# DiltheyLab/HLA-LA

Hardware: AMD Instinct MI355X
Metric: paired reads/sec aligned to PRG graph (higher is better)
Workload: dtype int32

## Files before the change

hla-la_amd/csrc/batch.h:

```cpp
#pragma once
#include "device_common.h"

namespace hlala {

template <template <class> class Ptr> struct DevBatchT {
    int n_pairs, n_reads, n_chains, stride;
    int from_seeds;
    int unpaired;
    Ptr<const int> read_off;
    Ptr<const uint8_t> read_bases;
    Ptr<const uint8_t> read_quals;
    Ptr<const int> chain_off;
    Ptr<const int> read_primary;
    Ptr<const int> chain_read;
    Ptr<const int> chain_contig;
    Ptr<const int> chain_pos;
    Ptr<const int> chain_offset;
    Ptr<const int> chain_as;
    Ptr<const uint8_t> chain_reverse;
    Ptr<const int> cigar_off;
    Ptr<const u32> cigar;
    Ptr<int> seed_status;
    Ptr<int> seed_ncols;
    Ptr<int> seed_begin;
// ... 40 lines not shown
    Ptr<int> order_hist;
    int order_shift, order_nb;
    int long_chunk_nodes, long_max_segs;
    int order_cost;
    Ptr<int> chain_row;
    int n_rows;
    Ptr<int> dp_blk;
    Ptr<int> dp_list;
    int dp_nblk;
    int dp_band;
    int dp_band_risky;
    int dp_jf;
    Ptr<void> dp_items;
    Ptr<int> dbg;
};
typedef DevBatchT<HostP> DevBatch;
typedef DevBatchT<GlobP> DevBatchG;
static_assert(sizeof(DevBatch) == sizeof(DevBatchG), "one layout");
__device__ __forceinline__ const DevBatchG& dev_view(const DevBatch* p) { return *(const DevBatchG*)p; }
enum { DESC_VALUE = 0, DESC_VIEW = 1, DESC_GENERIC = 2 };
template <int FORM, class D> __device__ __forceinline__ decltype(auto) desc_of(const D& byValue, const D* inMemory)
{
    if constexpr (FORM == DESC_VIEW) return dev_view(inMemory);
    else if constexpr (FORM == DESC_GENERIC) return (*inMemory);
    else return (byValue);
}

template <class BT> __device__ __forceinline__ int ordered_chains(const BT& B) { return B.chain_order ? __builtin_amdgcn_readfirstlane(B.order_hist[B.order_nb - 1]) : B.n_chains; }

template <class BT> __device__ __forceinline__ size_t row_base(const BT& B, int c) { return (size_t)(B.chain_row ? B.chain_row[c] : c) * (size_t)B.stride; }

enum { DPL_BAND16 = 0, DPL_BAND32 = 2, DPL_BAND64 = 4, DPL_JF = 6, DPL_GEN = 8, DPL_N = 10 };
__host__ __device__ inline int dpl_of_class(int cls) { return cls == 0 ? DPL_GEN : (cls == 1 ? DPL_JF : (cls == 2 ? DPL_BAND16 : (cls == 3 ? DPL_BAND32 : DPL_BAND64))); }
enum { WC_PAIR_MULTI = 40, WC_BAND_FETCH = 48, WC_FO_COUNT = 54, WC_FO_FETCH = 56, WC_BAND_FAILED = 58, WC_BAND_CALLS = 59, WC_JF_FAILED = 60, WC_BAND_WHY = 62, WC_BAND_TIED = 68,
       WC_N = 88 };
constexpr int BAND_MAXJ16 = 15, BAND_MAXJ32 = 31, BAND_MAXJ64 = 48;

enum {
    CNT_CHAINS_EXT = 0, CNT_DP_CALLS, CNT_DP_ITERS, CNT_DP_CELLS, CNT_SEED_COLS, CNT_OUT_COLS, CNT_EDGES, CNT_ERRORS, CNT_DP_SHARED
};

}
```

hla-la_amd/csrc/hlala_api.hip:

```cpp
#include <cmath>
#include <cstdio>
#include <cstring>
#include <cstdlib>
#include <algorithm>
#include <map>
#include <mutex>
#include <chrono>
#include <thread>
#include <set>
#include <string>
#include <unordered_map>
#include <vector>

#include "../../include/hlala_gpu.h"
#include "batch.h"
#include "flat_graph.hpp"
#include "host_internal.h"

#include "kernel_dp.hip"
#include "kernel_project.hip"
#include "kernel_order.hip"
#include "kernel_pair.hip"
#include "kernel_typer.hip"
#include "kernel_call.hip"
// ... 16 lines not shown

struct hlala_ctx {
    int device = 0;
    hipStream_t stream = nullptr;
    hipStream_t side = nullptr;
    hipStream_t up = nullptr, rs = nullptr, active = nullptr;
    int tail_pool_k = 1; std::vector<hlala_batch*> tail;
    hipEvent_t evSideTail = nullptr; bool sideTailValid = false;
    hlala_params params{};
    FlatGraph F;
    DevGraph G{};
    DevGraph* dG = nullptr;
    DevTables* dT = nullptr;
    double* d_islog = nullptr;
    long long* d_contig_off = nullptr; uint8_t* d_contig_seq = nullptr; int* d_contig_level = nullptr;
    int n_contigs = 0; std::vector<long long> contig_off;
    std::vector<void*> allocs;
    std::unordered_map<void*, size_t> block_bytes;
    std::multimap<size_t, void*> pool;
    size_t pool_bytes = 0;
    size_t pool_cap = (size_t)176 << 30;
    std::mutex pool_mu;
    std::set<struct hlala_batch*> batches;
    int jf_margin = 16;
    int stitch_by_row = 1;
    int stitch_draw = 12;
    bool side_after_pair = false;
    bool rows_all = false;
    bool band_risky = false;
    int band_grid = 0, band_margin = 8;
    char* tiny_slabs = nullptr; size_t tiny_slab_bytes = 0; int tiny_grid = 0; int jf_grid = 0;
    char* ext_slabs = nullptr; size_t ext_slab_bytes = 0; char* wide_slabs = nullptr; char* mid_slabs = nullptr; char* large_slabs = nullptr; size_t large_slab_bytes = 0; char* huge_slabs = nullptr; size_t huge_slab_bytes = 0; int huge_grid = 0; int ext_grid = 0; int wide_grid = 0; int broad_grid = 0; int retry_grid = 0; int stitch_grid = 0; int mid_grid = 0; size_t mid_slab_bytes = 0;
    char* proj_slabs = nullptr; size_t proj_slab_bytes = 0; int proj_grid = 0, pair_grid = 0, pair_lean_grid = 0;
    char* rethread_slabs = nullptr; size_t rethread_slab_bytes = 0; int rethread_grid = 0;
    double* pair_scratch = nullptr;
    char* proj_long_slabs = nullptr; size_t proj_long_slab_bytes = 0;
    void* create_scratch = nullptr; size_t create_scratch_bytes = 0; bool create_scratch_pinned = false;
    int long_chunk_nodes = 1 << 20, long_max_segs = 1 << 20;
    int order_cost = 0;
    int order_shift = 8, order_nb = 0;
    int* dbg_host = nullptr;
    int* d_cov = nullptr; int n_cov = 0; int* d_gene_first = nullptr; int* d_gene_last = nullptr; int n_genes = 0;
    struct KeptReads { uint8_t* store = nullptr; long long* start = nullptr; int* length = nullptr; int n = 0; };
    std::vector<KeptReads> kept;
    std::string err;
};

struct hlala_batch {
    hlala_ctx* ctx = nullptr;
    DevBatch B{};
    DevBatch* dB = nullptr;
    std::vector<void*> allocs;
    int staged = 0;
    bool prepared = false;
    int n_rows_host = 0;
    bool outputs_ready = false;
    bool side_used = false;
    bool side_pending = false;
    bool tail_pooled = false;
    bool side_inflight = false;
    hipEvent_t evDone = nullptr;
    hipEvent_t evMain = nullptr; bool mainValid = false;
    hipEvent_t ev[14]{}; hipEvent_t evC[7][2]{}; hipEvent_t evSide[8]{}; hipEvent_t evJF = nullptr;  hipEvent_t evBand[2]{};  bool band_used = false; bool eventsMade = false;
    uint32_t first_chain = 0;
    float ms[3] = {0, 0, 0};
};

// ... 329 lines not shown

    c->wide_grid = cus * 7;
    c->stitch_grid = cus * 20;
    if(const char* e = getenv("HLALA_STITCH_BY_ROW")) c->stitch_by_row = atoi(e) != 0;
    c->ext_slab_bytes = dp_slab_bytes<DpSmall>() > dp_slab_bytes<DpWide>() ? dp_slab_bytes<DpSmall>() : dp_slab_bytes<DpWide>();
    c->large_slab_bytes = dp_slab_bytes<DpLarge>() > dp_slab_bytes<DpBroad>() ? dp_slab_bytes<DpLarge>() : dp_slab_bytes<DpBroad>();
    c->huge_grid = cus / 4 > 0 ? cus / 4 : 1;
    c->huge_slab_bytes = dp_inmemory_bytes<DpHuge>();
    if((rc = slab_pool(&c->tiny_slabs, c->tiny_slab_bytes * (size_t)(64 / DpTiny::GW) * (size_t)std::max(c->tiny_grid, c->jf_grid), "16-lane DP slabs"))) return fail(rc);
    if((rc = slab_pool(&c->mid_slabs, c->mid_slab_bytes * (size_t)(64 / DpMid::GW) * (size_t)c->mid_grid, "32-lane DP slabs"))) return fail(rc);
    if((rc = slab_pool(&c->ext_slabs, c->ext_slab_bytes * (size_t)c->ext_grid, "64-lane DP slabs"))) return fail(rc);
    if((rc = slab_pool(&c->wide_slabs, c->ext_slab_bytes * (size_t)c->wide_grid, "wide-class DP slabs"))) return fail(rc);
    if((rc = slab_pool(&c->large_slabs, c->large_slab_bytes * (size_t)(c->broad_grid + c->retry_grid), "large-class DP slabs"))) return fail(rc);
    if((rc = slab_pool(&c->huge_slabs, c->huge_slab_bytes * (size_t)c->huge_grid, "in-memory DP class"))) return fail(rc);
    c->proj_grid = cus * (c->params.max_columns <= PROJ_CAP_SHORT ? 12 : 8); c->pair_grid = cus * 16; c->pair_lean_grid = cus * 24;
    { int rcp = dev_alloc(c, c->allocs, (size_t)2 * c->pair_grid * PAIR_COMB, &c->pair_scratch, false); if(rcp) return fail(rcp); }
    if(c->params.max_columns > PROJ_CAP) {
        c->proj_grid = cus * 20;
        c->proj_long_slab_bytes = proj_long_slab_bytes();
        c->stitch_draw = 1;
        if(device_malloc_retry(c->device, nullptr, (void**)&c->proj_long_slabs, c->proj_long_slab_bytes * (size_t)c->proj_grid) != hipSuccess) { c->err = "hipMalloc(long-read projection slabs) failed"; return fail(HLALA_E_DEVICE); }
        c->allocs.push_back(c->proj_long_slabs);
    }
    c->proj_slab_bytes = proj_slab_bytes_host(c->params.max_columns, F.max_nodes_per_level);
    if(device_malloc_retry(c->device, nullptr, (void**)&c->proj_slabs, c->proj_slab_bytes * (size_t)c->proj_grid) != hipSuccess) { c->err = "hipMalloc(projection slabs) failed"; return fail(HLALA_E_DEVICE); }
    c->allocs.push_back(c->proj_slabs);
    if(!c->proj_long_slabs) {
        const char* e = getenv("HLALA_RETHREAD");
        if(!(e && atoi(e) == 0)) {
            size_t ent = (size_t)c->params.max_columns * (size_t)RT_SN; if(ent < 1024) ent = 1024;
            c->rethread_slab_bytes = (ent * sizeof(ChoiceRec) + 255) & ~(size_t)255;
            if(c->rethread_slab_bytes > c->proj_slab_bytes) c->rethread_slab_bytes = c->proj_slab_bytes;
            c->rethread_grid = cus * 24;
            if(device_malloc_retry(c->device, nullptr, (void**)&c->rethread_slabs, c->rethread_slab_bytes * (size_t)c->rethread_grid) != hipSuccess) { c->err = "hipMalloc(re-threading slabs) failed"; return fail(HLALA_E_DEVICE); }
            c->allocs.push_back(c->rethread_slabs);
        }
    }
    { const char* e = getenv("HLALA_LOCALITY");
      if(!(e && atoi(e) == 0)) { int sh = 8; if(e && atoi(e) >= 2 && atoi(e) <= 20) sh = atoi(e); while((F.L >> sh) + 2 > 16384) sh++; c->order_shift = sh; c->order_nb = (F.L >> sh) + 2; } }
    if(const char* e = getenv("HLALA_LONG_CHUNK_NODES")) { const int v = atoi(e); if(v >= 1) c->long_chunk_nodes = v; }
    if(const char* e = getenv("HLALA_LONG_MAXSEGS")) { const int v = atoi(e); if(v >= 0) c->long_max_segs = v; }
    if(c->proj_long_slabs && c->order_nb > 0) { const char* e = getenv("HLALA_LONG_ORDER"); c->order_cost = (e && atoi(e) == 0) ? 0 : 1; }
    if(getenv("HLALA_DEBUG")) { if(hipMalloc((void**)&c->dbg_host, 8192 * sizeof(int)) != hipSuccess) c->dbg_host = nullptr; else { (void)hipMemset(c->dbg_host, 0, 8192 * sizeof(int)); c->allocs.push_back(c->dbg_host); } }
    if(hipEventCreateWithFlags(&c->evSideTail, hipEventDisableTiming) != hipSuccess) { c->err = "hipEventCreate failed"; return fail(HLALA_E_DEVICE); }
    { int prLow = 0, prHigh = 0; (void)hipDeviceGetStreamPriorityRange(&prLow, &prHigh);
      if(hipStreamCreateWithPriority(&c->up, hipStreamNonBlocking, prHigh) != hipSuccess || hipStreamCreateWithPriority(&c->rs, hipStreamNonBlocking, prHigh) != hipSuccess ||
         hipStreamCreateWithPriority(&c->side, hipStreamNonBlocking, prLow) != hipSuccess) { c->err = "hipStreamCreate failed"; return fail(HLALA_E_DEVICE); } }
    if(hipStreamSynchronize(c->active) != hipSuccess) { c->err = "upload failed"; return fail(HLALA_E_DEVICE); }
    { std::lock_guard<std::mutex> g(g_ctx_mu); g_ctxs.push_back(c); }
    *out = c;
    return HLALA_OK;
}

void hlala_destroy(hlala_ctx* c)
{
    if(!c) return;
    DEV_GUARD(c);
    { std::lock_guard<std::mutex> g(g_ctx_mu); g_ctxs.erase(std::remove(g_ctxs.begin(), g_ctxs.end(), c), g_ctxs.end()); }
    if(!c->tail.empty()) (void)flush_tail(c);
    for(hlala_batch* b : c->batches) b->ctx = nullptr;
    for(void* p : c->allocs) if(p) (void)hipFree(p);
    if(c->create_scratch) { if(c->create_scratch_pinned) (void)hipHostFree(c->create_scratch); else free(c->create_scratch); }
    for(hlala_ctx::KeptReads& kr : c->kept) { (void)hipFree(kr.store); (void)hipFree(kr.start); (void)hipFree(kr.length); }
    for(auto& kv : c->pool) (void)hipFree(kv.second);
    if(c->side) { (void)hipStreamSynchronize(c->side); (void)hipStreamDestroy(c->side); }
    if(c->up) { (void)hipStreamSynchronize(c->up); (void)hipStreamDestroy(c->up); }
// ... 322 lines not shown
{
    DEV_GUARD(c);
    if(!c || !b) return HLALA_E_ARG;
    { int rj = join_side(c, b); if(rj) return rj; }
    if(b->B.from_seeds) { c->err = "batch was created from seeds: stage A not available"; return HLALA_E_STATE; }
    { int re = batch_events(c, b); if(re) return re; }
    { int ro = ensure_outputs(c, b); if(ro) return ro; }
    DevBatch& B = b->B;
    HIP_TRY(c, hipMemsetAsync(B.work_counter, 0, WC_N * sizeof(int), c->active));
    HIP_TRY(c, hipMemsetAsync(B.counters, 0, 32 * sizeof(u64), c->active));
    HIP_TRY(c, hipEventRecord(b->ev[0], c->active));
    if(B.n_chains > 0) {
        int threads = 256, blocks = (B.n_reads + threads - 1) / threads;
        if(!b->prepared && B.order_hist) HIP_TRY(c, hipMemsetAsync(B.order_hist, 0, ((size_t)B.order_nb + 1) * sizeof(int), c->active));
        if(!b->prepared) hipLaunchKernelGGL(k_filter_chains, dim3(blocks), dim3(threads), 0, c->active, c->dG, b->dB, c->d_contig_off, c->d_contig_level);
        if(!b->prepared && B.order_hist) {
            hipLaunchKernelGGL(k_order_scan, dim3(1), dim3(ORDER_SCAN_THREADS), 0, c->active, B.order_hist, B.order_nb);
            hipLaunchKernelGGL(k_order_scatter, dim3((B.n_chains + 255) / 256), dim3(256), 0, c->active, b->dB);
            int rco = check_launch(c, "k_order_scatter"); if(rco) return rco;
        }
        int grid = B.n_chains < c->proj_grid ? B.n_chains : c->proj_grid;
        if(c->proj_long_slabs)
            hipLaunchKernelGGL((k_project_chains<ProjLdsLong>), dim3(grid), dim3(64), 0, c->active, c->G, b->B, c->dG, b->dB, c->d_contig_off, c->d_contig_seq, c->d_contig_level,
                               c->proj_slabs, c->proj_slab_bytes, c->proj_long_slabs, c->proj_long_slab_bytes, 0);
        else
            if(c->params.max_columns <= PROJ_CAP_SHORT)
                hipLaunchKernelGGL((k_project_chains<ProjLdsShort>), dim3(grid), dim3(64), 0, c->active, c->G, b->B, c->dG, b->dB, c->d_contig_off, c->d_contig_seq, c->d_contig_level,
                                   c->proj_slabs, c->proj_slab_bytes, (char*)nullptr, (size_t)0, c->rethread_slabs ? 1 : 0);
            else
                hipLaunchKernelGGL((k_project_chains<ProjLds>), dim3(grid), dim3(64), 0, c->active, c->G, b->B, c->dG, b->dB, c->d_contig_off, c->d_contig_seq, c->d_contig_level,
                               c->proj_slabs, c->proj_slab_bytes, (char*)nullptr, (size_t)0, c->rethread_slabs ? 1 : 0);
        int rc = check_launch(c, "k_project_chains"); if(rc) return rc;
        if(c->rethread_slabs) {
            hipLaunchKernelGGL(k_rethread_chains, dim3(c->rethread_grid), dim3(64), 0, c->active, c->dG, b->dB, c->rethread_slabs, c->rethread_slab_bytes);
            rc = check_launch(c, "k_rethread_chains"); if(rc) return rc;
        }
    }
    HIP_TRY(c, hipEventRecord(b->ev[1], c->active));
    b->staged |= 1;
    return mark_main(c, b);
}

static int extend_impl(hlala_ctx* c, hlala_batch* b, bool fused, int phase = 0);
int hlala_extend_chains(hlala_ctx* c, hlala_batch* b) { return extend_impl(c, b, false); }

static int extend_impl(hlala_ctx* c, hlala_batch* b, bool fused, int phase)
{
    DEV_GUARD(c);
    if(!c || !b) return HLALA_E_ARG;
    if(!(b->staged & 1)) { c->err = "hlala_extend_chains before seed chains exist"; return HLALA_E_STATE; }
    const bool sidePartOnly = phase == 2 || phase == 4;
    if(!sidePartOnly) { int rj = join_side(c, b); if(rj) return rj; }
    { int re = batch_events(c, b); if(re) return re; }
    DevBatch& B = b->B;
    if(B.unpaired || B.from_seeds || B.n_pairs <= 0 || B.n_chains <= 0) { fused = false; if(sidePartOnly) return HLALA_OK; phase = 0; }
    const bool mainPart = !sidePartOnly;
    if(mainPart) {
    b->side_used = false; b->side_pending = false;
    if(B.n_pairs > 0) HIP_TRY(c, hipMemsetAsync(B.pair_deferred, 0, (size_t)B.n_pairs, c->active));
    HIP_TRY(c, hipMemsetAsync(B.work_counter + 1, 0, sizeof(int), c->active));
    HIP_TRY(c, hipMemsetAsync(B.work_counter + 4, 0, (WC_N - 4) * sizeof(int), c->active));
    if(B.from_seeds) HIP_TRY(c, hipMemsetAsync(B.counters, 0, 32 * sizeof(u64), c->active));
    HIP_TRY(c, hipEventRecord(b->ev[2], c->active));
    }
    if(B.n_chains > 0) {
        DpItem* items = (DpItem*)B.dp_items;
        const u32 seed = c->params.rng_seed + 2u * b->first_chain;
// ... 1413 lines not shown
```

hla-la_amd/csrc/kernel_project.hip:

```cpp
#include "batch.h"
#include "../../include/hlala_gpu.h"

namespace hlala {

constexpr int PROJ_CAP   = 512;
constexpr int PROJ_NODES = 512;
constexpr int PROJ_SN    = 640;
constexpr int PROJ_SE    = 768;
constexpr int PROJ_SEGMAX = 24;

struct ChoiceRec { int eid; short fromz; short S; };

constexpr int RT_SN = 416;
constexpr int RT_CE = 512;
constexpr int CHAIN_RETHREAD_PENDING = 64;


template <int CAP_, int SN_, int SE_>
struct __align__(16) ProjLdsT {
    static constexpr int CAP = CAP_, SN = SN_, SE = SE_; static constexpr bool LONG = false;
    typedef unsigned short LvT;
    LvT lvl[2][CAP_];
    unsigned char g[2][CAP_], s[2][CAP_];
    short Srow[2][PROJ_NODES];
    unsigned short sLev[CAP_ + 2];
    unsigned short sIn[SN_ + 1];
    unsigned short sChoice[SN_];
    static constexpr int CE = (3 * SE_) / 4;
    union {
        struct { unsigned short sFrom[SE_];
                 unsigned char sLab[SE_]; };
        u32 eRec[CE];
    };
    u32 colInfo[CAP_];
    unsigned short segStart[CAP_ + 2];
    u64 mGap[CAP_ / 64], mDef[CAP_ / 64], mSeq[CAP_ / 64];
    int err, n, startRaw, stopRaw, tmp0, tmp1;
    __device__ __forceinline__ short* sflat() { return &Srow[0][0]; }
};
typedef ProjLdsT<PROJ_CAP, PROJ_SN, PROJ_SE> ProjLds;
constexpr int PROJ_CAP_SHORT = 384;
typedef ProjLdsT<PROJ_CAP_SHORT, 416, 544> ProjLdsShort;

constexpr int PROJL_CAP = 16384;
constexpr int PROJL_SN  = 49152;
constexpr int PROJL_SE  = 57344;
constexpr int PROJL_LONGSEG = 32;
struct __align__(16) ProjLdsLong {
// ... 801 lines not shown
                                    const int sp = P.Srow[rowP][fz];
                                    if(sp < 0) continue;
                                    const int lab = (int)((r >> 18) & 0xFFu);
                                    if(seedIsMatch && lab != sc) continue;
                                    const int cd = sp + (lab == sc ? 1 : 0);
                                    if(cd > best) { best = cd; bestE = e - eL0; bestFrom = fz; }
                                }
                                if(!par) edgesTouched += (u64)(e1 - e0);
                                P.Srow[1 - rowP][z] = (short)best;
                                chw[tBase + t - nb] = best >= 0 ? ((u32)bestFrom | ((u32)bestE << 16)) : 0xFFFFFFFFu;
                                if(best >= 0) reached = true;
                            }
                            prevFast = false;
                        }
                        if(!__ballot(reached)) { if(lane == 0) PJ_FAIL(HLALA_CHAIN_ERR_INPUT); stop = true; break; }
                        rowP = 1 - rowP;
                        LSYNC();
                    }
                    WSYNC();
                    if(PJ_FINE && B.dbg) { tSub[0] += tC1 - tC0; tSub[1] += clock64() - tC1; tSub[2]++; tSub[3] += cnt; }
                    if(stop) break;
                    a = b + 1;
                }
                }
            }
            chunked = !PL::LONG && !par && windowed && defCount == nDef;
            if(runLevels) { }
            else if(chunked) {
                staged_rows<7>(lane, nDef + 1, 64, [&](int i) { int2 r; r.x = G.in_off[nodeBase + P.sLev[i + 1]]; r.y = (!PL::LONG && i < nDef) ? (int)G.level_fast[level0 + i + 1] : 0; return r; },
                               [&](int i, int2 r) { P.segStart[i] = (unsigned short)(r.x - eBase); if(!PL::LONG && i < nDef && r.y) P.colInfo[i] |= (u32)r.y << 25; });
                WSYNC();
                if constexpr (!PL::LONG) if(deferRethread) {
                    int mxN = nb - nodeBase, mxE = 0;
                    for(int i = lane; i < nDef; i += 64) { mxN = max(mxN, (int)P.sLev[i + 2] - (int)P.sLev[i + 1]); mxE = max(mxE, (int)P.segStart[i + 1] - (int)P.segStart[i]); }
                    mxN = wave_max_i32(mxN); mxE = wave_max_i32(mxE);
                    if(mxN <= RT_SN && mxE <= RT_CE) {
                        deferred = true;
                        const size_t cb = row_base(B, c);
                        for(int j = lane; j < n1; j += 64) { B.seed_level[cb + j] = LC::get(P.lvl[cur][j], lvBase); B.seed_g[cb + j] = P.g[cur][j]; B.seed_s[cb + j] = P.s[cur][j]; }
                        for(int i = lane; i < nDef; i += 64) B.seed_edge[cb + i] = (int)P.colInfo[i];
                        unsigned short* lvRow = (unsigned short*)(B.ext_level + cb); unsigned short* sgRow = (unsigned short*)(B.ext_edge + cb);
                        for(int i = lane; i <= nDef + 1; i += 64) lvRow[i] = P.sLev[i];
                        for(int i = lane; i <= nDef; i += 64) sgRow[i] = P.segStart[i];
                        if(lane == 0) {
                            B.seed_ncols[c] = n1; B.seed_begin[c] = P.startRaw; B.seed_end[c] = P.stopRaw; B.seed_removed[c] = removed; B.seed_status[c] = CHAIN_RETHREAD_PENDING;
                            int* st = (int*)B.dp_items + (size_t)c * 16;
                            *(int4*)st = make_int4(level0, nDef, nodeBase, nb); st[4] = eBase; st[5] = n1;
                        }
                    }
                }
                const int nbR = nb - nodeBase;
                int a = deferred ? nDef : 0;
                while(a < nDef && PJ_OK()) {
                    const int cand = a + lane;
                    const bool fits = cand < nDef && (PL::LONG || lane < 62) && ((int)P.sLev[cand + 2] - (int)P.sLev[a + 1]) <= PL::SN && ((int)P.segStart[cand + 1] - (int)P.segStart[a]) <= PL::CE;
                    const u64 fm = __ballot(fits);
                    const int cnt = (fm == ~0ull) ? 64 : (__ffsll((long long)~fm) - 1);
                    if(cnt == 0) {
                        if(lane == 0) P.sChoice[nChunks] = (unsigned short)(a | 0x8000);
                        nChunks++;
                        const u32 ci = P.colInfo[a];
                        const unsigned char sc = (unsigned char)((ci >> 16) & 0xFFu); const bool seedIsMatch = ((ci >> 24) & 1u) != 0;
                        const int tb = nodeBase + P.sLev[a + 1], tm = (int)P.sLev[a + 2] - (int)P.sLev[a + 1], fb = nodeBase + P.sLev[a];
                        if(tm > PROJ_NODES) { if(lane == 0) PJ_FAIL(HLALA_CHAIN_ERR_FRONTIER); break; }
                        int anyReached = 0;
                        for(int z = lane; z < tm; z += 64) {
                            const int node = tb + z;
                            int best = -1, bestE = -1, bestFrom = -1;
                            const int e0 = G.in_off[node], e1 = G.in_off[node + 1];
                            for(int e = e0; e < e1; e++) {
                                const int fz = G.in_from[e] - fb; const int sp = P.Srow[rowP][fz];
                                if(sp < 0) continue;
                                const unsigned char lab = G.in_label[e];
                                if(seedIsMatch && lab != sc) continue;
                                const int cd = sp + (lab == sc ? 1 : 0);
                                if(cd > best) { best = cd; bestE = e - eBase; bestFrom = fz; }
                            }
                            edgesTouched += (u64)(e1 - e0);
// ... 313 lines not shown
            if(k >= 25) {
                { const int q = atomicAdd(&B.dbg[4318], 1); if(q < 300) { int* r = B.dbg + 5000 + 10 * q; r[0] = c; r[1] = dbgN[0]; r[2] = dbgN[1]; r[3] = dbgN[2]; r[4] = dbgN[3]; r[5] = dbgN[4]; r[6] = dbgN[5]; r[7] = dbgN[6]; r[8] = (int)(cyc >> 16); r[9] = dbgN[7] | ((int)((tPh[0] >> 20) & 0x7FFFF) << 8); } }
                atomicAdd(&B.dbg[4319], 1);
                for(int i = 0; i < 6; i++) atomicAdd(&B.dbg[4320 + i], (int)((tPh[i + 1] - tPh[i]) >> 12));
                for(int i = 0; i < 12; i++) atomicAdd(&B.dbg[4330 + i], (int)((tFine[i] - tFine0[i]) >> 12));
                for(int i = 0; i < 4; i++) atomicAdd(&B.dbg[4344 + i], (int)((tSub[i] - tSub0[i]) >> (i < 2 ? 12 : 0)));
            }
        }
        {
            int e = wave_sum_i32((int)edgesTouched);
            accEdges += (u64)e;
        }
        WSYNC();
        if(!PJ_OK() && lane == 0) { B.seed_status[c] = P.err; B.seed_ncols[c] = 0; }
        }
        WSYNC();
        }
    }
    if(lane == 0) { if(accCols) atomicAdd(&B.counters[CNT_SEED_COLS], accCols); if(accEdges) atomicAdd(&B.counters[CNT_EDGES], accEdges); }
#ifndef HLALA_DP_TIMING
    if(B.dbg && lane == 0) { for(int i = 0; i < 6; i++) atomicAdd(&B.counters[16 + i], (u64)tAcc[i]); atomicAdd(&B.counters[23], (u64)tAcc[6]); }
    if(B.dbg && lane == 0) for(int i = 0; i < 4; i++) atomicAdd(&B.counters[24 + i], (u64)tSub[i]);
    if constexpr (PL::LONG && PJ_FINE) if(B.dbg && lane == 0) for(int i = 0; i < 12; i++) atomicAdd(&B.dbg[4300 + i], (int)(tFine[i] >> 12));
#endif
}

struct __align__(16) RethreadLds {
    u32 eRec[RT_CE];
    unsigned short sIn[RT_SN + 2];
    short Srow[2][PROJ_NODES];
    unsigned short pick[PROJ_CAP];
    u64 chunkStart[PROJ_CAP / 64];
};

__global__ __launch_bounds__(64, 6) void k_rethread_chains(const DevGraph* __restrict__ Gp, const DevBatch* __restrict__ Bp, char* slabs, size_t slabBytes)
{
    const DevGraphG& G = dev_view(Gp);
    const DevBatchG& B = dev_view(Bp);
    __shared__ RethreadLds P;
    const int lane = lane_id();
    u32* const ch = (u32*)(slabs + (size_t)blockIdx.x * slabBytes);
    const int stride = B.stride;
    u64 accCols = 0, accEdges = 0;
    const int nWork = ordered_chains(B);
    for(;;) {
        constexpr int RT_DRAW = 16;
        int c0 = 0;
        if(lane == 0) c0 = atomicAdd(&B.work_counter[3], RT_DRAW);
        c0 = __builtin_amdgcn_readfirstlane(c0);
        if(c0 >= nWork) break;
        const int cq = (lane < RT_DRAW && c0 + lane < nWork) ? (B.chain_order ? B.chain_order[c0 + lane] : c0 + lane) : -1;
        u64 pend = __ballot(cq >= 0 && B.seed_status[cq] == CHAIN_RETHREAD_PENDING);
        for(; pend; pend &= pend - 1) {
            const int c = __builtin_amdgcn_readlane(cq, __ffsll((long long)pend) - 1);
            const size_t cb = row_base(B, c);
            const int* st = (const int*)B.dp_items + (size_t)c * 16;
            int sv = lane < 6 ? st[lane] : 0;
            const int level0 = __builtin_amdgcn_readlane(sv, 0), nDef = __builtin_amdgcn_readlane(sv, 1), nodeBase = __builtin_amdgcn_readlane(sv, 2), nb = __builtin_amdgcn_readlane(sv, 3),
                      eBase = __builtin_amdgcn_readlane(sv, 4), n1 = __builtin_amdgcn_readlane(sv, 5);
            (void)level0;
            const unsigned short* lvRow = (const unsigned short*)(B.ext_level + cb); const unsigned short* sgRow = (const unsigned short*)(B.ext_edge + cb);
            const int* ciRow = B.seed_edge + cb;
            const int nbR = nb - nodeBase;
            for(int z = lane; z < nbR; z += 64) P.Srow[0][z] = 0;
            if(lane < PROJ_CAP / 64) P.chunkStart[lane] = 0;
            WSYNC();
            int rowP = 0, err = 0;
            u64 edgesTouched = 0;
            int a = 0;
            while(a < nDef && !err) {
                const int i0 = a + lane;
                const int lvA = i0 <= nDef + 1 ? (int)lvRow[i0] : 0, lvC = i0 + 2 <= nDef + 1 ? (int)lvRow[i0 + 2] : 0;
                const int sgA = i0 <= nDef ? (int)sgRow[i0] : 0, sgB = i0 + 1 <= nDef ? (int)sgRow[i0 + 1] : 0;
                const u32 ciReg = i0 < nDef ? (u32)ciRow[i0] : 0u;
                const int lvA1 = __builtin_amdgcn_readlane(lvA, 1), sgA0 = __builtin_amdgcn_readlane(sgA, 0);
                const bool fits = i0 < nDef && lane < 62 && (lvC - lvA1) <= RT_SN && (sgB - sgA0) <= RT_CE;
                const u64 fm = __ballot(fits);
                const int cnt = __ffsll((long long)~fm) - 1;
                if(cnt == 0) { err = HLALA_CHAIN_ERR_FRONTIER; break; }
                const int b = a + cnt - 1;
                if(lane == 0) P.chunkStart[a >> 6] |= 1ull << (a & 63);
                const int tBase = lvA1, nT = __builtin_amdgcn_readlane(lvA, cnt + 1) - tBase, eC = sgA0, nE = __builtin_amdgcn_readlane(sgA, cnt) - eC;
                const int lvReg = lvA, sgReg = sgA - eC;
                {
                    constexpr int UE = RT_CE / 64, UN = (RT_SN + 1 + 63) / 64;
// ... 118 lines not shown
                int z = zsel;
                for(int bb = nDef - 1; bb >= 0; ) {
                    int w = bb >> 6; u64 m = P.chunkStart[w] & (~0ull >> (63 - (bb & 63)));
                    while(m == 0) { w--; m = P.chunkStart[w]; }
                    const int aa = w * 64 + 63 - __clzll((long long)m);
                    const int i0 = aa + lane;
                    const int lvA = i0 <= nDef + 1 ? (int)lvRow[i0] : 0;
                    const u32 ciReg = i0 <= bb ? (u32)ciRow[i0] : 0u;
                    const int tBase = __builtin_amdgcn_readlane(lvA, 1), nT = __builtin_amdgcn_readlane(lvA, bb - aa + 2) - tBase;
                    {
                        constexpr int UN = (RT_SN + 63) / 64;
                        u32 vr[UN];
                        #pragma unroll
                        for(int u = 0; u < UN; u++) { const int t = lane + 64 * u; if(t < nT) vr[u] = ch[tBase + t - nbR]; }
                        #pragma unroll
                        for(int u = 0; u < UN; u++) { const int t = lane + 64 * u; if(t < nT) P.eRec[t] = vr[u]; }
                    }
                    WSYNC();
                    for(int i = bb; i >= aa; i--) {
                        const int col = (int)((u32)__builtin_amdgcn_readlane((int)ciReg, i - aa) & 0xFFFFu), lvI = __builtin_amdgcn_readlane(lvA, i - aa + 1);
                        if(lane == 0) { const u32 r = P.eRec[lvI - tBase + z]; P.pick[col] = (unsigned short)(r >> 16); z = (int)(short)(r & 0xFFFFu); }
                    }
                    WSYNC();
                    bb = aa - 1;
                }
                staged_rows<6>(lane, n1, 64, [&](int j) { const unsigned short pe = P.pick[j]; FromLab r; r.from = -1; r.lab = '_';
                                                          if(pe != 0xFFFF) { r.from = G.in_eid[eBase + pe]; r.lab = G.in_label[eBase + pe]; } return r; },
                               [&](int j, FromLab r) { B.seed_edge[cb + j] = r.from; B.seed_g[cb + j] = r.lab; });
                if(lane == 0) { B.seed_status[c] = HLALA_CHAIN_OK; accCols += (u64)n1; }
            } else if(lane == 0) { B.seed_status[c] = err; B.seed_ncols[c] = 0; }
            accEdges += edgesTouched;
            WSYNC();
        }
    }
    accCols = wave_sum_u64(accCols); accEdges = wave_sum_u64(accEdges);
    if(lane == 0) { if(accCols) atomicAdd(&B.counters[CNT_SEED_COLS], accCols); if(accEdges) atomicAdd(&B.counters[CNT_EDGES], accEdges); }
}

}
```

include/hlala_gpu.h:

```cpp
#ifndef HLALA_GPU_H_
#define HLALA_GPU_H_

#include <stddef.h>
#include <stdint.h>

#ifdef __cplusplus
extern "C" {
#endif

#define HLALA_OK              0
#define HLALA_E_ARG          -1
#define HLALA_E_DEVICE       -2
#define HLALA_E_GRAPH        -3
#define HLALA_E_CAPACITY     -4
#define HLALA_E_STATE        -5

#define HLALA_CHAIN_OK             0
#define HLALA_CHAIN_SKIP_STRAND    1
#define HLALA_CHAIN_SKIP_DUP       2
#define HLALA_CHAIN_ERR_COLUMNS   -1
#define HLALA_CHAIN_ERR_FRONTIER  -2
#define HLALA_CHAIN_ERR_INPUT     -3

typedef struct {
// ... 421 lines not shown
    int32_t unaccounted_min_coverage;
    int32_t pairs_file_done;
    double  unaccounted_min_fraction;
    const hlala_unit_stats_out* unit_stats;
    const uint8_t* unit_mask;
    int32_t n_units;
    int32_t reserved2;
    double  insert_mean, insert_sd, min_mapq, min_weighted_ok;
} hlala_locus_report_in;
typedef struct {
    double  locus_coverage, first_decile_coverage, minimum_coverage, avg_column_error, min_column_p;
    int64_t bases_used;
    int32_t n_columns_unaccounted, n_utilized_reads, n_piled_positions, reserved;
} hlala_locus_report_out;
int  hlala_typer_begin_output(const char* out_dir, double unaccounted_min_fraction);
int  hlala_locus_write_files(const hlala_locus* l, const hlala_locus_report_in* in, const char* out_dir, hlala_locus_report_out* out);
int  hlala_locus_write_pairs_file(const hlala_locus* l, int32_t n_clusters, const int32_t* order, const double* p_normalized, const double* pair_ll,
                                  const double* mis_avg, const char* out_dir);
int  hlala_typer_end_output(const char* out_dir, const char* loci_comma_separated, int32_t very_conservative_read_likelihoods);

int  hlala_kat_phred(hlala_ctx* ctx, int n, const double* p_correct, uint8_t* phred_out,
                     const uint8_t* phred_in, double* p_out);
int  hlala_kat_rand_r(hlala_ctx* ctx, int n, uint32_t* seeds_inout, int32_t* values_out);
int  hlala_kat_exp(hlala_ctx* ctx, int n, const double* x, double* exp_x);

int  hlala_abi_sizeof(const char* struct_name);

#define HLALA_ABI_VERSION 6
int  hlala_abi_version(void);
#define HLALA_DEBUG_WC_N           88
#define HLALA_DEBUG_WC_BAND_FETCH  48
#define HLALA_DEBUG_WC_BAND_WHY    62
#define HLALA_DEBUG_WC_BAND_TIED   68
int  hlala_debug_work_counters(hlala_ctx* ctx, hlala_batch* batch, int* out, int capacity);
int  hlala_debug_dp_items(hlala_ctx* ctx, hlala_batch* batch, int* items_out, long long items_capacity_bytes, int* retry_out, long long retry_capacity_bytes);
int  hlala_debug_counters(hlala_ctx* ctx, hlala_batch* batch, unsigned long long* out32);
int  hlala_debug_buffer(hlala_ctx* ctx, int* out8192, int clear);
int  hlala_debug_memory(hlala_ctx* ctx, hlala_batch* batch, unsigned long long* out4);

#define HLALA_BUILD_AGENT_RELEASE 2
int  hlala_build_flags(void);

#ifdef __cplusplus
}
#endif
#endif
```

Measured before the change: 5.657 million.

## Rethread two narrow chains per wave using 32-lane halves

The projection kernel now tags deferred chains whose frontier, edge span and column count are small (and not on the slow path) as narrow. The rethreading kernel then processes two narrow chains at once, one per 32-lane half of the wave, with separate LDS buffers placed in a union so the total LDS size does not grow. This targets lanes left idle when a small chain occupies a full 64-lane wave. In exchange it adds lockstep control flow for both halves, divergence when the two chains have different lengths, and a halved slab per chain. The path can be turned off with an environment variable.

```diff
diff --git a/hla-la_amd/csrc/batch.h b/hla-la_amd/csrc/batch.h
--- a/hla-la_amd/csrc/batch.h
+++ b/hla-la_amd/csrc/batch.h
@@ -96,7 +96,7 @@
 
 enum { DPL_BAND16 = 0, DPL_BAND32 = 2, DPL_BAND64 = 4, DPL_JF = 6, DPL_GEN = 8, DPL_N = 10 };
 __host__ __device__ inline int dpl_of_class(int cls) { return cls == 0 ? DPL_GEN : (cls == 1 ? DPL_JF : (cls == 2 ? DPL_BAND16 : (cls == 3 ? DPL_BAND32 : DPL_BAND64))); }
-enum { WC_PAIR_MULTI = 40, WC_BAND_FETCH = 48, WC_FO_COUNT = 54, WC_FO_FETCH = 56, WC_BAND_FAILED = 58, WC_BAND_CALLS = 59, WC_JF_FAILED = 60, WC_BAND_WHY = 62, WC_BAND_TIED = 68,
+enum { WC_RT_PAIRED = 72, WC_RT_HALF = 73, WC_PAIR_MULTI = 40, WC_BAND_FETCH = 48, WC_FO_COUNT = 54, WC_FO_FETCH = 56, WC_BAND_FAILED = 58, WC_BAND_CALLS = 59, WC_JF_FAILED = 60, WC_BAND_WHY = 62, WC_BAND_TIED = 68,
        WC_N = 88 };
 constexpr int BAND_MAXJ16 = 15, BAND_MAXJ32 = 31, BAND_MAXJ64 = 48;
 
diff --git a/hla-la_amd/csrc/hlala_api.hip b/hla-la_amd/csrc/hlala_api.hip
--- a/hla-la_amd/csrc/hlala_api.hip
+++ b/hla-la_amd/csrc/hlala_api.hip
@@ -72,7 +72,7 @@
     char* tiny_slabs = nullptr; size_t tiny_slab_bytes = 0; int tiny_grid = 0; int jf_grid = 0;
     char* ext_slabs = nullptr; size_t ext_slab_bytes = 0; char* wide_slabs = nullptr; char* mid_slabs = nullptr; char* large_slabs = nullptr; size_t large_slab_bytes = 0; char* huge_slabs = nullptr; size_t huge_slab_bytes = 0; int huge_grid = 0; int ext_grid = 0; int wide_grid = 0; int broad_grid = 0; int retry_grid = 0; int stitch_grid = 0; int mid_grid = 0; size_t mid_slab_bytes = 0;
     char* proj_slabs = nullptr; size_t proj_slab_bytes = 0; int proj_grid = 0, pair_grid = 0, pair_lean_grid = 0;
-    char* rethread_slabs = nullptr; size_t rethread_slab_bytes = 0; int rethread_grid = 0;
+    char* rethread_slabs = nullptr; size_t rethread_slab_bytes = 0; int rethread_grid = 0; int rethread_pairs = 0;
     double* pair_scratch = nullptr;
     char* proj_long_slabs = nullptr; size_t proj_long_slab_bytes = 0;
     void* create_scratch = nullptr; size_t create_scratch_bytes = 0; bool create_scratch_pinned = false;
@@ -468,6 +468,8 @@
             c->rethread_slab_bytes = (ent * sizeof(ChoiceRec) + 255) & ~(size_t)255;
             if(c->rethread_slab_bytes > c->proj_slab_bytes) c->rethread_slab_bytes = c->proj_slab_bytes;
             c->rethread_grid = cus * 24;
+            { const char* ep = getenv("HLALA_RETHREAD_PAIRS"); size_t need = c->proj_slab_bytes / sizeof(ChoiceRec); if(need > (size_t)RT_PAIR_NODES) need = (size_t)RT_PAIR_NODES;
+              c->rethread_pairs = !(ep && atoi(ep) == 0) && c->rethread_slab_bytes / 8 >= need ? 1 : 0; }
             if(device_malloc_retry(c->device, nullptr, (void**)&c->rethread_slabs, c->rethread_slab_bytes * (size_t)c->rethread_grid) != hipSuccess) { c->err = "hipMalloc(re-threading slabs) failed"; return fail(HLALA_E_DEVICE); }
             c->allocs.push_back(c->rethread_slabs);
         }
@@ -856,7 +858,7 @@
                                c->proj_slabs, c->proj_slab_bytes, (char*)nullptr, (size_t)0, c->rethread_slabs ? 1 : 0);
         int rc = check_launch(c, "k_project_chains"); if(rc) return rc;
         if(c->rethread_slabs) {
-            hipLaunchKernelGGL(k_rethread_chains, dim3(c->rethread_grid), dim3(64), 0, c->active, c->dG, b->dB, c->rethread_slabs, c->rethread_slab_bytes);
+            hipLaunchKernelGGL(k_rethread_chains, dim3(c->rethread_grid), dim3(64), 0, c->active, c->dG, b->dB, c->rethread_slabs, c->rethread_slab_bytes, c->rethread_pairs);
             rc = check_launch(c, "k_rethread_chains"); if(rc) return rc;
         }
     }
diff --git a/hla-la_amd/csrc/kernel_project.hip b/hla-la_amd/csrc/kernel_project.hip
--- a/hla-la_amd/csrc/kernel_project.hip
+++ b/hla-la_amd/csrc/kernel_project.hip
@@ -14,6 +14,13 @@
 constexpr int RT_SN = 416;
 constexpr int RT_CE = 512;
 constexpr int CHAIN_RETHREAD_PENDING = 64;
+constexpr int CHAIN_RETHREAD_NARROW = 65;
+constexpr int RT_PAIR_E = 32;
+constexpr int RT_PAIR_SN = 208;
+constexpr int RT_PAIR_COLS = 384;
+constexpr int RT_PAIR_NODES = RT_PAIR_COLS * RT_PAIR_E;
+constexpr int RT_PAIR_CE = 256;
+constexpr int RT_PAIR_LV = 30;
 
 
 template <int CAP_, int SN_, int SE_>
@@ -881,8 +888,10 @@
                 WSYNC();
                 if constexpr (!PL::LONG) if(deferRethread) {
                     int mxN = nb - nodeBase, mxE = 0;
-                    for(int i = lane; i < nDef; i += 64) { mxN = max(mxN, (int)P.sLev[i + 2] - (int)P.sLev[i + 1]); mxE = max(mxE, (int)P.segStart[i + 1] - (int)P.segStart[i]); }
+                    bool slow = false;
+                    for(int i = lane; i < nDef; i += 64) { mxN = max(mxN, (int)P.sLev[i + 2] - (int)P.sLev[i + 1]); mxE = max(mxE, (int)P.segStart[i + 1] - (int)P.segStart[i]); slow |= ((P.colInfo[i] >> 25) & 3u) != 1u; }
                     mxN = wave_max_i32(mxN); mxE = wave_max_i32(mxE);
+                    const bool narrow = !__ballot(slow) && mxE <= RT_PAIR_E && mxN <= RT_PAIR_SN && n1 <= RT_PAIR_COLS && chCount <= RT_PAIR_NODES;
                     if(mxN <= RT_SN && mxE <= RT_CE) {
                         deferred = true;
                         const size_t cb = row_base(B, c);
@@ -892,7 +901,7 @@
                         for(int i = lane; i <= nDef + 1; i += 64) lvRow[i] = P.sLev[i];
                         for(int i = lane; i <= nDef; i += 64) sgRow[i] = P.segStart[i];
                         if(lane == 0) {
-                            B.seed_ncols[c] = n1; B.seed_begin[c] = P.startRaw; B.seed_end[c] = P.stopRaw; B.seed_removed[c] = removed; B.seed_status[c] = CHAIN_RETHREAD_PENDING;
+                            B.seed_ncols[c] = n1; B.seed_begin[c] = P.startRaw; B.seed_end[c] = P.stopRaw; B.seed_removed[c] = removed; B.seed_status[c] = narrow ? CHAIN_RETHREAD_NARROW : CHAIN_RETHREAD_PENDING;
                             int* st = (int*)B.dp_items + (size_t)c * 16;
                             *(int4*)st = make_int4(level0, nDef, nodeBase, nb); st[4] = eBase; st[5] = n1;
                         }
@@ -1272,12 +1281,30 @@
     unsigned short pick[PROJ_CAP];
     u64 chunkStart[PROJ_CAP / 64];
 };
-
-__global__ __launch_bounds__(64, 6) void k_rethread_chains(const DevGraph* __restrict__ Gp, const DevBatch* __restrict__ Bp, char* slabs, size_t slabBytes)
+struct __align__(16) RethreadLdsPair {
+    u32 eRec[2][RT_PAIR_CE];
+    short Srow[2][2][RT_PAIR_SN];
+    unsigned short pick[2][RT_PAIR_COLS];
+    u64 chunkStart[2][RT_PAIR_COLS / 64];
+};
+union RethreadLdsU { RethreadLds one; RethreadLdsPair two; };
+static_assert(sizeof(RethreadLdsU) == sizeof(RethreadLds), "the paired form must not add LDS: 24 waves per CU");
+
+__device__ __forceinline__ int rt_half(int v, int i, int h) { const int a = __builtin_amdgcn_readlane(v, i), b = __builtin_amdgcn_readlane(v, 32 + i); return h ? b : a; }
+#define RT_HALF(v, i) rt_half((v), (i), h)
+__device__ __forceinline__ int half_max_i32(int v)
+{
+    #pragma unroll
+    for(int o = 16; o >= 1; o >>= 1) v = max(v, __shfl_xor(v, o));
+    return v;
+}
+
+__global__ __launch_bounds__(64, 6) void k_rethread_chains(const DevGraph* __restrict__ Gp, const DevBatch* __restrict__ Bp, char* slabs, size_t slabBytes, int pairs)
 {
     const DevGraphG& G = dev_view(Gp);
     const DevBatchG& B = dev_view(Bp);
-    __shared__ RethreadLds P;
+    __shared__ RethreadLdsU PU;
+    RethreadLds& P = PU.one;
     const int lane = lane_id();
     u32* const ch = (u32*)(slabs + (size_t)blockIdx.x * slabBytes);
     const int stride = B.stride;
@@ -1290,7 +1317,9 @@
         c0 = __builtin_amdgcn_readfirstlane(c0);
         if(c0 >= nWork) break;
         const int cq = (lane < RT_DRAW && c0 + lane < nWork) ? (B.chain_order ? B.chain_order[c0 + lane] : c0 + lane) : -1;
-        u64 pend = __ballot(cq >= 0 && B.seed_status[cq] == CHAIN_RETHREAD_PENDING);
+        const int stq = cq >= 0 ? B.seed_status[cq] : 0;
+        u64 narrow = pairs ? __ballot(stq == CHAIN_RETHREAD_NARROW) : 0ull;
+        u64 pend = __ballot(stq == CHAIN_RETHREAD_PENDING || stq == CHAIN_RETHREAD_NARROW) & ~narrow;
         for(; pend; pend &= pend - 1) {
             const int c = __builtin_amdgcn_readlane(cq, __ffsll((long long)pend) - 1);
             const size_t cb = row_base(B, c);
@@ -1475,6 +1504,164 @@
             accEdges += edgesTouched;
             WSYNC();
         }
+        while(narrow) {
+            RethreadLdsPair& Q = PU.two;
+            const int h = lane >> 5, hl = lane & 31;
+            const int cA = __builtin_amdgcn_readlane(cq, __ffsll((long long)narrow) - 1); narrow &= narrow - 1;
+            int cB = -1;
+            if(narrow) { cB = __builtin_amdgcn_readlane(cq, __ffsll((long long)narrow) - 1); narrow &= narrow - 1; }
+            const int cH = h ? cB : cA;
+            const bool act = cH >= 0;
+            const size_t cb = act ? row_base(B, cH) : 0;
+            const int* st = (const int*)B.dp_items + (size_t)(act ? cH : 0) * 16;
+            const int sv = (act && hl < 6) ? st[hl] : 0;
+            const int nDefA = __builtin_amdgcn_readlane(sv, 1), nDefB = __builtin_amdgcn_readlane(sv, 33);
+            const int nDef = h ? nDefB : nDefA, nbR = RT_HALF(sv, 3) - RT_HALF(sv, 2), eBase = RT_HALF(sv, 4), n1 = RT_HALF(sv, 5);
+            const unsigned short* lvRow = (const unsigned short*)(B.ext_level + cb); const unsigned short* sgRow = (const unsigned short*)(B.ext_edge + cb);
+            const int* ciRow = B.seed_edge + cb;
+            u32* const chH = ch + (h ? slabBytes / 8 : 0);
+            for(int z = hl; z < nbR; z += 32) Q.Srow[h][0][z] = 0;
+            if(hl < RT_PAIR_COLS / 64) Q.chunkStart[h][hl] = 0;
+            WSYNC();
+            int aA = 0, aB = 0, errA = 0, errB = 0, rowPA = 0, rowPB = 0;
+            u64 edgesTouched = 0;
+            for(;;) {
+                const bool runA = aA < nDefA && !errA, runB = aB < nDefB && !errB;
+                if(!runA && !runB) break;
+                const bool run = h ? runB : runA;
+                const int a = h ? aB : aA;
+                const int i0 = a + hl;
+                const int lvA = (run && i0 <= nDef + 1) ? (int)lvRow[i0] : 0, lvC = (run && i0 + 2 <= nDef + 1) ? (int)lvRow[i0 + 2] : 0;
+                const int sgA = (run && i0 <= nDef) ? (int)sgRow[i0] : 0, sgB = (run && i0 + 1 <= nDef) ? (int)sgRow[i0 + 1] : 0;
+                const u32 ciReg = (run && i0 < nDef) ? (u32)ciRow[i0] : 0u;
+                const int lvA1 = RT_HALF(lvA, 1), sgA0 = RT_HALF(sgA, 0);
+                const bool fits = run && i0 < nDef && hl < RT_PAIR_LV && (lvC - lvA1) <= RT_PAIR_SN && (sgB - sgA0) <= RT_PAIR_CE;
+                const u64 fm = __ballot(fits);
+                const int cntA = __ffs((int)~(u32)fm) - 1, cntB = __ffs((int)~(u32)(fm >> 32)) - 1;
+                if(runA && cntA == 0) errA = HLALA_CHAIN_ERR_FRONTIER;
+                if(runB && cntB == 0) errB = HLALA_CHAIN_ERR_FRONTIER;
+                if((runA && cntA == 0) || (runB && cntB == 0)) continue;
+                const int cnt = min(runA ? cntA : 64, runB ? cntB : 64);
+                if(hl == 0 && run) Q.chunkStart[h][a >> 6] |= 1ull << (a & 63);
+                const int eC = sgA0, nE = RT_HALF(sgA, cnt) - eC;
+                const int lvReg = lvA, sgReg = sgA - eC;
+                staged_rows<4>(hl, run ? nE : 0, 32, [&](int e) { return G.in_rec[eBase + eC + e]; }, [&](int e, u32 r) { Q.eRec[h][e] = r; });
+                WSYNC();
+                bool liveA = runA, liveB = runB;
+                bool prevFast = false;
+                int sReg = -1;
+                int eL0 = 0, eL1 = RT_HALF(sgReg, 1);
+                u32 recN = (run && hl < eL1) ? Q.eRec[h][hl] : 0u;
+                for(int k = 0; k < cnt; k++) {
+                    const u32 ciA = (u32)__builtin_amdgcn_readlane((int)ciReg, k), ciB = (u32)__builtin_amdgcn_readlane((int)ciReg, 32 + k);
+                    const u32 ci = h ? ciB : ciA;
+                    const int sc = (int)((ci >> 16) & 0xFFu); const bool seedIsMatch = ((ci >> 24) & 1u) != 0;
+                    const int l1 = RT_HALF(lvReg, k + 1);
+                    const int nEl = eL1 - eL0;
+                    const int maxd = __builtin_amdgcn_readfirstlane(max(liveA ? (int)((ciA >> 27) & 7u) : 0, liveB ? (int)((ciB >> 27) & 7u) : 0));
+                    const bool live = h ? liveB : liveA;
+                    const int rowP = h ? rowPB : rowPA;
+                    const u32 rec = recN;
+                    int eL2 = eL1;
+                    if(k + 1 < cnt) { eL2 = RT_HALF(sgReg, k + 2); recN = (live && hl < eL2 - eL1) ? Q.eRec[h][eL1 + hl] : 0u; }
+                    const bool mine = live && hl < nEl;
+                    int sp;
+                    if(prevFast) sp = __builtin_amdgcn_ds_bpermute((int)(((u32)(lane & 32) + ((rec >> 9) & 31u)) << 2), sReg);
+                    else sp = (int)Q.Srow[h][rowP][rec & 511u];
+                    const int m = (int)((rec >> 18) & 0xFFu) == sc ? 1 : 0;
+                    const int cand = (mine && sp >= 0 && (m || !seedIsMatch)) ? sp + m + 1 : 0;
+                    const int key = (cand << 15) | ((31 - hl) << 9) | (int)(rec & 511u);
+                    const int pos = (int)((rec >> 15) & 7u);
+                    int bk = key, kj = key;
+                    for(int j = 1; j <= maxd; j++) { kj = __builtin_amdgcn_update_dpp(0, kj, 0x138, 0xF, 0xF, false); if(pos >= j) bk = max(bk, kj); }
+                    const bool last = mine && (rec & (1u << 28)) != 0;
+                    const u64 lastMask = __ballot(last);
+                    const int best = (bk >> 15) - 1;
+                    sReg = best;
+                    bool reached = false;
+                    if(last) {
+                        const int tzA = (int)__builtin_amdgcn_mbcnt_lo((u32)lastMask, 0u), tzB = (int)__builtin_amdgcn_mbcnt_hi((u32)(lastMask >> 32), 0u);
+                        const int tz = h ? tzB : tzA;
+                        Q.Srow[h][1 - rowP][tz] = (short)best;
+                        chH[l1 + tz - nbR] = best >= 0 ? ((u32)(bk & 511) | ((u32)(eC + eL0 + 31 - ((bk >> 9) & 63)) << 16)) : 0xFFFFFFFFu;
+                        reached = best >= 0;
+                    }
+                    if(hl == 0 && live) edgesTouched += (u64)nEl;
+                    prevFast = true;
+                    const u64 rm = __ballot(reached);
+                    if(liveA && (u32)rm == 0u) { errA = HLALA_CHAIN_ERR_INPUT; liveA = false; }
+                    if(liveB && (u32)(rm >> 32) == 0u) { errB = HLALA_CHAIN_ERR_INPUT; liveB = false; }
+                    if(liveA) rowPA ^= 1;
+                    if(liveB) rowPB ^= 1;
+                    eL0 = eL1; eL1 = eL2;
+                    if(!liveA && !liveB) break;
+                    LSYNC();
+                }
+                WSYNC();
+                if(runA) aA += cnt;
+                if(runB) aB += cnt;
+            }
+            const int err = h ? errB : errA;
+            const bool ok = act && !err;
+            {
+                int tmL = 0;
+                if(ok) tmL = (int)lvRow[nDef + 1] - (int)lvRow[nDef];
+                const short* lastS = Q.Srow[h][h ? rowPB : rowPA];
+                int bestS = -1;
+                for(int z = hl; z < tmL; z += 32) bestS = max(bestS, (int)lastS[z]);
+                bestS = half_max_i32(bestS);
+                int zsel = 0x7FFFFFFF;
+                for(int z = hl; z < tmL; z += 32) if(lastS[z] == bestS) zsel = min(zsel, z);
+                zsel = -half_max_i32(-zsel);
+                for(int j = hl; j < (ok ? n1 : 0); j += 32) Q.pick[h][j] = 0xFFFF;
+                WSYNC();
+                int z = zsel;
+                int bbA = errA ? -1 : nDefA - 1, bbB = errB ? -1 : nDefB - 1;
+                while(bbA >= 0 || bbB >= 0) {
+                    const int bb = h ? bbB : bbA;
+                    const bool on = bb >= 0;
+                    int aa = 0;
+                    if(on) {
+                        int w = bb >> 6; u64 m = Q.chunkStart[h][w] & (~0ull >> (63 - (bb & 63)));
+                        while(m == 0) { w--; m = Q.chunkStart[h][w]; }
+                        aa = w * 64 + 63 - __clzll((long long)m);
+                    }
+                    const int aaA = __builtin_amdgcn_readlane(aa, 0), aaB = __builtin_amdgcn_readlane(aa, 32);
+                    const int i0 = aa + hl;
+                    const int lvA = (on && i0 <= nDef + 1) ? (int)lvRow[i0] : 0;
+                    const u32 ciReg = (on && i0 <= bb) ? (u32)ciRow[i0] : 0u;
+                    const int lenA = bbA >= 0 ? bbA - aaA + 1 : 0, lenB = bbB >= 0 ? bbB - aaB + 1 : 0;
+                    const int tBase = RT_HALF(lvA, 1);
+                    const int nTA = __builtin_amdgcn_readlane(lvA, lenA + 1), nTB = __builtin_amdgcn_readlane(lvA, 32 + lenB + 1);
+                    const int nT = (h ? nTB : nTA) - tBase;
+                    staged_rows<4>(hl, on ? nT : 0, 32, [&](int t) { return chH[tBase + t - nbR]; }, [&](int t, u32 r) { Q.eRec[h][t] = r; });
+                    WSYNC();
+                    const int steps = max(lenA, lenB);
+                    for(int s = 0; s < steps; s++) {
+                        const int kA = lenA - 1 - s, kB = lenB - 1 - s;
+                        const u32 cwA = (u32)__builtin_amdgcn_readlane((int)ciReg, max(kA, 0)), cwB = (u32)__builtin_amdgcn_readlane((int)ciReg, 32 + max(kB, 0));
+                        const int lvIA = __builtin_amdgcn_readlane(lvA, max(kA, 0) + 1), lvIB = __builtin_amdgcn_readlane(lvA, 32 + max(kB, 0) + 1);
+                        if(hl == 0 && (h ? kB : kA) >= 0) {
+                            const int col = (int)((h ? cwB : cwA) & 0xFFFFu), lvI = h ? lvIB : lvIA;
+                            const u32 r = Q.eRec[h][lvI - tBase + z]; Q.pick[h][col] = (unsigned short)(r >> 16); z = (int)(short)(r & 0xFFFFu);
+                        }
+                    }
+                    WSYNC();
+                    if(bbA >= 0) bbA = aaA - 1;
+                    if(bbB >= 0) bbB = aaB - 1;
+                }
+                staged_rows<3>(hl, ok ? n1 : 0, 32, [&](int j) { const unsigned short pe = Q.pick[h][j]; FromLab r; r.from = -1; r.lab = '_';
+                                                                 if(pe != 0xFFFF) { r.from = G.in_eid[eBase + pe]; r.lab = G.in_label[eBase + pe]; } return r; },
+                               [&](int j, FromLab r) { B.seed_edge[cb + j] = r.from; B.seed_g[cb + j] = r.lab; });
+            }
+            if(hl == 0 && act) {
+                if(!err) { B.seed_status[cH] = HLALA_CHAIN_OK; accCols += (u64)n1; }
+                else { B.seed_status[cH] = err; B.seed_ncols[cH] = 0; }
+            }
+            if(lane == 0) atomicAdd(&B.work_counter[cB >= 0 ? WC_RT_PAIRED : WC_RT_HALF], cB >= 0 ? 2 : 1);
+            accEdges += edgesTouched;
+            WSYNC();
+        }
     }
     accCols = wave_sum_u64(accCols); accEdges = wave_sum_u64(accEdges);
     if(lane == 0) { if(accCols) atomicAdd(&B.counters[CNT_SEED_COLS], accCols); if(accEdges) atomicAdd(&B.counters[CNT_EDGES], accEdges); }
diff --git a/include/hlala_gpu.h b/include/hlala_gpu.h
--- a/include/hlala_gpu.h
+++ b/include/hlala_gpu.h
@@ -477,6 +477,7 @@
 #define HLALA_DEBUG_WC_BAND_FETCH  48
 #define HLALA_DEBUG_WC_BAND_WHY    62
 #define HLALA_DEBUG_WC_BAND_TIED   68
+#define HLALA_DEBUG_WC_RT_PAIRED   72
 int  hlala_debug_work_counters(hlala_ctx* ctx, hlala_batch* batch, int* out, int capacity);
 int  hlala_debug_dp_items(hlala_ctx* ctx, hlala_batch* batch, int* items_out, long long items_capacity_bytes, int* retry_out, long long retry_capacity_bytes);
 int  hlala_debug_counters(hlala_ctx* ctx, hlala_batch* batch, unsigned long long* out32);
```

Result: no change. 5.652 million (-0.1%).
